# qpc001/ORB_SLAM2_Commit

Hardware: AMD Instinct MI355X
Metric: frames/sec ORB extract+match (2k kp) + LocalBA iters/sec, KITTI-00 stereo (higher is better)
Workload: dtype u8; 1 GPU; KITTI-00 stereo 1241x376, 2000 features, extract L+R + ComputeStereoMatches; batch_frames_per_gpu=256, global_batch_frames=256, nlevels=8, parallelism=frame-sharded x1, batches_in_flight=4

## Files before the change

### include/orbx_debug.h

```cpp
#ifndef ORBX_DEBUG_H
#define ORBX_DEBUG_H
#include "orbx.h"
#ifdef __cplusplus
extern "C" {
#endif

enum {
  ORBX_DBG_BLUR_LEVEL = 1,
  ORBX_DBG_CELL_COUNTS = 2,
  ORBX_DBG_CELL_TABLE = 3,
  ORBX_DBG_CANDIDATES = 4,
  ORBX_DBG_OCT_COUNTS = 5,
  ORBX_DBG_OCT_OUT = 6,
  ORBX_DBG_LEVEL_INFO = 7
};

long long orbx_debug_copy(orbx_extractor* h, int what, int image, int arg, void* dst, size_t cap);

enum {
  ORBX_LP_LEVELS = 1,
  ORBX_LP_RESIZE = 2,
  ORBX_LP_BOUNDS = 3,
  ORBX_LP_GRIDS = 4,
  ORBX_LP_REMAP = 5,
  ORBX_LP_XTAB = 6,
  ORBX_LP_YTAB = 7,
  ORBX_LP_PATH = 8
};
long long orbx_debug_launch_plan(const orbx_extractor_params* params, int width, int height, int what, int a0,
                                 int a1, int a2, long long* dst, size_t cap);

orbx_status orbx_debug_stereo_keypoints(orbx_extractor* left, orbx_extractor* right, const orbx_keypoint* kpsL,
                                        const uint8_t* descL, int nL, const orbx_keypoint* kpsR, const uint8_t* descR,
                                        int nR, float bf, float baseline, float* uRight, float* depth, int32_t* sad,
                                        int32_t* nmatches);
int orbx_debug_stereo_keypoints_check(const orbx_keypoint* kps, int n, int nlevels, int width, int height);

double orbx_debug_atan2_det(double y, double x);

int orbx_debug_lm_step(double state[5], int counts[2], double tempChi, double scale, int ok2, int cube_kind,
                       int ops);

int orbx_debug_exp(const double* x, int n, double* y, int device);
int orbx_debug_sim3_exp(const double update[7], const double S[8], int fix_scale, double out[8], int device);

int orbx_debug_log(const double* x, int n, double* y, int device);
int orbx_debug_acos(const double* x, int n, double* y, int device);
int orbx_debug_sim3_log(const double* S, int n, double* out, int32_t* branch, int device);
int orbx_debug_essgraph_linearize(const orbx_essential_graph_problem* problem, double* meas, double* err,
                                  double* J0, double* J1, double* H, double* b, int device);
int orbx_debug_essgraph_solve(const orbx_essential_graph_problem* problem, const double* H, const double* b,
                              double lambda, double* x, int32_t* ok, int device);
int orbx_debug_essgraph_phases(const orbx_essential_graph_problem* problem, const orbx_essential_graph_result* result,
                               double phase_ms[3], long long* envelope_blocks, int device);

int orbx_debug_ldlt(const double* S, const double* b, int N, double* x, int reps, float* ms);
int orbx_debug_ldlt_ex(const double* S, const double* b, int N, double* x, int reps, float* ms, int kind,
                       unsigned long long* stamps);

#define ORBX_BA_LDLT_AUTO 0
// ... 46 lines not shown
```

### orb_slam2_commit_amd/csrc/capi.hip

```cpp
#include <hip/hip_runtime.h>

#include <algorithm>
#include <cmath>
#include <cstring>
#include <map>
#include <memory>
#include <new>
#include <utility>
#include <string>
#include <vector>

#include "../../include/orbx.h"
#include "orbx_internal.h"
#include "orbx_scratch.h"
#include "orbx_stereo.h"
#include "orbx_prof.h"
#include "orbx_bow.h"

namespace orbx {
hipError_t upload_constants(const int* umax16, const int* gauss7);
hipError_t launch_blur(const Geometry& Gh, const Geometry* Gd, const int* tile_level, const BatchPtrs& B, int n_img,
                       hipStream_t st);
hipError_t launch_extract_stages(const Geometry& Gh, const Geometry* Gd, const CellInfo* cells, const int* tile_level,
                                 const LaunchPlan& LP, const BatchPtrs& B, int n_img, orbx_keypoint* kps, uint8_t* desc, int32_t* counts,
                                 int kp_cap, hipStream_t st, StageTimer* T);
size_t octree_smem_host(int NC, int cell_cap, int kcap);
hipError_t octree_set_smem_limit(size_t bytes);
}

using namespace orbx;

namespace {

inline int round_even(float v) { return (int)std::nearbyintf(v); }

constexpr size_t kInSlack = 4;

template <class T>
struct DevBuf {
  T* p = nullptr;
  size_t n = 0;
  ~DevBuf() { release(); }
  void release() {
    if (p) (void)hipFree(p);
    p = nullptr;
    n = 0;
  }
  hipError_t ensure(size_t count) {
    if (count <= n && p) return hipSuccess;
    release();
    size_t c = std::max<size_t>(count, 1);
    hipError_t e = hipMalloc((void**)&p, c * sizeof(T));
    if (e == hipSuccess) n = c;
    return e;
  }
};

struct Tables {
  std::vector<float> scale, inv_scale, sigma2, inv_sigma2;
  std::vector<int> nfeat;
// ... 220 lines not shown
        if (sx + 1 >= sw && sx >= sw - 1) { fx = 0; sx = sw - 1; }
        ResizeX X;
        X.sx0 = sx;
        X.sx1 = std::min(sx + 1, sw - 1);
        X.a0 = (int16_t)round_even((1.f - fx) * 2048);
        X.a1 = (int16_t)round_even(fx * 2048);
        if (sx + 1 >= sw) {
          X.a0 = 2048;
          X.a1 = 0;
        }
        P.xt.push_back(X);
      }
      L.ytab_off = (int)P.yt.size();
      for (int dy = 0; dy < dh; dy++) {
        float fy = (float)((dy + 0.5) * scale_y - 0.5);
        int sy = (int)std::floor(fy);
        fy -= sy;
        ResizeY Y;
        Y.sy0 = std::min(std::max(sy, 0), sh - 1);
        Y.sy1 = std::min(std::max(sy + 1, 0), sh - 1);
        Y.b0 = (int16_t)round_even((1.f - fy) * 2048);
        Y.b1 = (int16_t)round_even(fy * 2048);
        P.yt.push_back(Y);
      }
    }
  }
  {
    auto layout = [&](int wmax, int hmax, Geometry::FastGroup& g) {
      g.s = wmax + 6 <= 40 ? 40 : wmax + 6 <= 48 ? 48 : 80;
      g.rp = wmax <= 32 ? 2 : 1;
      g.tile_bytes = ((hmax + 6) * g.s + 15) & ~15;
      g.map_bytes = ((hmax + 2) * g.s + 15) & ~15;
      g.smem = g.tile_bytes + g.map_bytes + 2 * wmax * hmax;
    };
    constexpr int kFastLdsFit = 5 * 1024;
    int split = 0, wa = 1, ha = 1;
    for (int l = 0; l < p.nlevels; l++) {
      Geometry::FastGroup g{};
      layout(std::max(wa, lv_wmax[l]), std::max(ha, lv_hmax[l]), g);
      if (g.smem > kFastLdsFit) break;
      wa = std::max(wa, lv_wmax[l]);
      ha = std::max(ha, lv_hmax[l]);
      split = l + 1;
    }
    if (split == 0 || split == p.nlevels) split = p.nlevels;
    int wb = 1, hb = 1;
    for (int l = split; l < p.nlevels; l++) {
      wb = std::max(wb, lv_wmax[l]);
      hb = std::max(hb, lv_hmax[l]);
    }
    G.n_fg = 0;
    if (split == p.nlevels) {
      int w = 1, h = 1;
      for (int l = 0; l < p.nlevels; l++) {
        w = std::max(w, lv_wmax[l]);
        h = std::max(h, lv_hmax[l]);
      }
      layout(w, h, G.fg[0]);
      G.fg[0].c0 = 0;
      G.fg[0].c1 = (int)P.cells.size();
      G.n_fg = 1;
    } else {
      layout(wa, ha, G.fg[0]);
      G.fg[0].c0 = 0;
      G.fg[0].c1 = G.lv[split].cell_begin;
      layout(wb, hb, G.fg[1]);
      G.fg[1].c0 = G.lv[split].cell_begin;
      G.fg[1].c1 = (int)P.cells.size();
      G.n_fg = 2;
    }
  }
  G.rz_rows = 1;
  G.rz_stride = 16;
  for (int l = 1; l < G.nlevels; l++) {
    const LevelGeom& L = G.lv[l];
    P.rzb_x[l] = (int)P.rzb.size();
    for (int ox = 0; ox < L.w; ox += kRzTW) {
      const int sx0 = P.xt[L.xtab_off + ox].sx0, sx1 = P.xt[L.xtab_off + std::min(ox + kRzTW, L.w) - 1].sx1;
      P.rzb.push_back(make_int2(sx0, sx1));
      G.rz_stride = std::max(G.rz_stride, (sx1 - sx0 + 1 + 15) / 16 * 16);
    }
    P.rzb_y[l] = (int)P.rzb.size();
    for (int oy = 0; oy < L.h; oy += kRzTH) {
      const int sy0 = P.yt[L.ytab_off + oy].sy0, sy1 = P.yt[L.ytab_off + std::min(oy + kRzTH, L.h) - 1].sy1;
      P.rzb.push_back(make_int2(sy0, sy1));
      G.rz_rows = std::max(G.rz_rows, sy1 - sy0 + 1);
    }
  }
  if (G.rz_rows > kRzMaxRows || (size_t)G.rz_rows * (G.rz_stride + 2 * kRzTW) > 64 * 1024) return ORBX_ERR_SIZE;
  P.rzb_n = (int)P.rzb.size();
  for (int l = 1; l < G.nlevels; l++) {
    const LevelGeom& L = G.lv[l];
    P.strip[l] = strip_resize_ok(P, l);
    if (!P.strip[l]) continue;
    P.rsb_x[l] = (int)P.rzb.size();
    for (int ox = 0; ox < L.w; ox += kRsTW)
      P.rzb.push_back(make_int2(P.xt[L.xtab_off + ox].sx0, P.xt[L.xtab_off + std::min(ox + kRsTW, L.w) - 1].sx1));
    P.rsb_y[l] = (int)P.rzb.size();
    for (int oy = 0; oy < L.h; oy += kRsTH)
      P.rzb.push_back(make_int2(P.yt[L.ytab_off + oy].sy0, P.yt[L.ytab_off + std::min(oy + kRsTH, L.h) - 1].sy1));
  }
  G.rz_lc = 0;
  while ((1 << G.rz_lc) < G.rz_stride / 16) G.rz_lc++;
// ... 787 lines not shown
      break;
    }
    case ORBX_DBG_CANDIDATES: {
      std::vector<uint32_t> raw((size_t)G.cand_total);
      if (hipMemcpy(raw.data(), h->cand.p + (size_t)image * G.cand_total, raw.size() * 4, hipMemcpyDeviceToHost) !=
          hipSuccess)
        return ORBX_ERR_HIP;
      std::vector<uint32_t> logical;
      logical.reserve(raw.size());
      for (const CellInfo& c : P.cells)
        for (int q = 0; q < c.cap; q++) logical.push_back(raw[cell_slot(c, q)]);
      static_assert(sizeof(uint32_t) == sizeof(int), "host staging is int words");
      host.resize(logical.size());
      std::memcpy(host.data(), logical.data(), logical.size() * 4);
      device_src = false;
      break;
    }
    case ORBX_DBG_OCT_COUNTS:
      src = h->oct_count.p + (size_t)image * G.nlevels;
      bytes = sizeof(int) * G.nlevels;
      break;
    case ORBX_DBG_OCT_OUT:
      src = h->oct.p + (size_t)image * G.oct_total;
      bytes = sizeof(uint32_t) * G.oct_total;
      break;
    case ORBX_DBG_LEVEL_INFO:
      for (int l = 0; l < G.nlevels; l++) {
        const LevelGeom& L = G.lv[l];
        int v[8] = {L.w, L.h, L.cell_begin, L.cell_end, L.oct_off, L.oct_cap, L.nfeat, L.nIni};
        host.insert(host.end(), v, v + 8);
      }
      device_src = false;
      break;
    default:
      return ORBX_ERR_ARG;
  }
  if (!device_src) {
    bytes = host.size() * sizeof(int);
    if (dst) std::memcpy(dst, host.data(), std::min(bytes, cap));
    return (long long)bytes;
  }
  if (dst && cap) {
    if (hipMemcpy(dst, src, std::min(bytes, cap), hipMemcpyDeviceToHost) != hipSuccess) return ORBX_ERR_HIP;
  }
  return (long long)bytes;
}

extern "C" int orbx_debug_stereo_keypoints_check(const orbx_keypoint* kps, int n, int nlevels, int width,
                                                 int height) {
  if (n < 0 || (n > 0 && !kps) || nlevels < 1 || nlevels > kMaxLevelsPlan || width <= 0 || height <= 0)
    return ORBX_ERR_ARG;
  for (int i = 0; i < n; i++) {
    const orbx_keypoint& k = kps[i];
    if (k.octave < 0 || k.octave >= nlevels) return ORBX_ERR_ARG;
    if (!std::isfinite(k.x) || !std::isfinite(k.y) || std::signbit(k.x) || std::signbit(k.y)) return ORBX_ERR_ARG;
    if (!(k.x < (float)width) || !(k.y < (float)height)) return ORBX_ERR_ARG;
  }
  return ORBX_OK;
}

extern "C" orbx_status orbx_debug_stereo_keypoints(orbx_extractor* left, orbx_extractor* right,
                                                   const orbx_keypoint* kpsL, const uint8_t* descL, int nL,
                                                   const orbx_keypoint* kpsR, const uint8_t* descR, int nR, float bf,
                                                   float baseline, float* uRight, float* depth, int32_t* sad,
                                                   int32_t* nmatches) {
  if (!uRight || !depth || !sad || !nmatches || nL < 0 || nR < 0) return ORBX_ERR_ARG;
// ... 63 lines not shown
  }
  if (!params_ok(params) || width <= 0 || height <= 0) return ORBX_ERR_ARG;
  Plan P;
  const orbx_status s = build_plan(*params, make_tables(*params), width, height, P);
  if (s != ORBX_OK) return s;
  build_launch_plan(P, P.xt.data(), P.yt.data(), P.rzb.data(), P.LP);
  const Geometry& G = P.G;
  switch (what) {
    case ORBX_LP_LEVELS:
      for (int l = 0; l < G.nlevels; l++) {
        const LevelGeom& L = G.lv[l];
        out.insert(out.end(), {L.w, L.h, L.off, L.boff, L.bstride, L.tile_begin, L.tiles_x, L.tiles_y});
      }
      break;
    case ORBX_LP_RESIZE:
      for (int l = 1; l < G.nlevels; l++) {
        const ResizeDesc& D = P.LP.rz[l];
        out.insert(out.end(), {D.sw, D.sh, D.dw, D.dh, D.src_off, D.dst_off, D.pyr_bytes, D.X - P.xt.data(),
                               D.Y - P.yt.data(), D.bx - P.rzb.data(), D.by - P.rzb.data(), D.stride, D.rows, D.lc,
                               (D.dw + kRzTW - 1) / kRzTW, (D.dh + kRzTH - 1) / kRzTH});
      }
      break;
    case ORBX_LP_BOUNDS:
      for (int i = 0; i < P.rzb_n; i++) out.insert(out.end(), {P.rzb[i].x, P.rzb[i].y});
      break;
    case ORBX_LP_PATH:
      for (int l = 1; l < G.nlevels; l++) {
        const bool f = P.strip[l];
        const int tw = f ? kRsTW : kRzTW, th = f ? kRsTH : kRzTH;
        out.insert(out.end(), {f ? 1 : 0, (G.lv[l].w + tw - 1) / tw, (G.lv[l].h + th - 1) / th, tw, th,
                               f ? kRsStride : G.rz_stride, f ? kRsRows : G.rz_rows, f ? kRsR : 0});
      }
      break;
    case ORBX_LP_GRIDS: {
      if (a0 < 1) return ORBX_ERR_ARG;
      for (int l = 1; l < G.nlevels; l++)
        out.insert(out.end(), {(G.lv[l].w + kRzTW - 1) / kRzTW, (G.lv[l].h + kRzTH - 1) / kRzTH, a0});
      out.insert(out.end(), {G.ntiles, a0, 1});
      break;
    }
    case ORBX_LP_XTAB:
    case ORBX_LP_YTAB: {
      if (a0 < 1 || a0 >= G.nlevels) return ORBX_ERR_ARG;
      const LevelGeom& L = G.lv[a0];
      if (what == ORBX_LP_XTAB)
        for (int i = 0; i < L.w; i++) {
          const ResizeX& X = P.xt[L.xtab_off + i];
          out.insert(out.end(), {X.sx0, X.sx1, X.a0, X.a1});
        }
      else
        for (int i = 0; i < L.h; i++) {
          const ResizeY& Y = P.yt[L.ytab_off + i];
          out.insert(out.end(), {Y.sy0, Y.sy1, Y.b0, Y.b1});
        }
      break;
    }
    default:
      return ORBX_ERR_ARG;
  }
  return done();
}

typedef unsigned int u32x4 __attribute__((ext_vector_type(4)));
__global__ __launch_bounds__(256) void k_hbm_copy(u32x4* __restrict__ dst, const u32x4* __restrict__ src, size_t n) {
  const size_t i = (size_t)blockIdx.x * 256 + threadIdx.x;
  if (i < n) __builtin_nontemporal_store(__builtin_nontemporal_load(src + i), dst + i);
// ... 27 lines not shown
```

### orb_slam2_commit_amd/csrc/extract.hip

```cpp
#include <hip/hip_runtime.h>

#include <utility>

#include "orbx_device.h"
#include "orbx_internal.h"
#include "orbx_prof.h"

namespace orbx {

__constant__ float c_pattern_f[1024] = {
#include "brief_pattern_31.inc"
};
__constant__ uint4 c_icmask[64];
__constant__ double c_sincos[23] = {
    6.36619772367581382433e-01,
    1.57079632673412561417e+00,
    6.07710050650619224932e-11,
    1.0 / 51090942171709440000.0, -1.0 / 121645100408832000.0, 1.0 / 355687428096000.0,
    -1.0 / 1307674368000.0,       1.0 / 6227020800.0,           -1.0 / 39916800.0,
    1.0 / 362880.0,               -1.0 / 5040.0,                1.0 / 120.0,
    -1.0 / 6.0,
    1.0 / 2432902008176640000.0,  -1.0 / 6402373705728000.0,    1.0 / 20922789888000.0,
    -1.0 / 87178291200.0,         1.0 / 479001600.0,            -1.0 / 3628800.0,
    1.0 / 40320.0,                -1.0 / 720.0,                 1.0 / 24.0,
// ... 352 lines not shown
  RZ_PROBE_WRITE(ts1 - ts0, 0, ts2 - ts1, ts3 - ts2, 1);
}

__constant__ int c_gauss[7];

__device__ __forceinline__ int reflect101(int p, int n) {
  if (n == 1) return 0;
  while ((unsigned)p >= (unsigned)n) p = p < 0 ? -p : 2 * n - 2 - p;
  return p;
}

constexpr int kBIn = kBlurTileW + 16;
constexpr int kBStrip = 16;
#ifndef ORBX_BLUR_WPE
#define ORBX_BLUR_WPE 7
#endif
__global__ __launch_bounds__(BS, ORBX_BLUR_WPE) void k_blur(const Geometry* __restrict__ G, const int* __restrict__ tile_level,
                                                            BatchPtrs B, XcdRemap R) {
  constexpr int TR = kBlurTileH + 6;
  __shared__ __align__(16) uint8_t tin[(TR + 1) * kBIn];
  const int2 bi = xcd_block2(R);
  const int tile = bi.x, img = bi.y, tid = threadIdx.x;
  const int l = tile_level[tile];
  const LevelGeom& L = G->lv[l];
  const int t = tile - L.tile_begin;
  const int x0 = (t % L.tiles_x) * kBlurTileW, y0 = (t / L.tiles_x) * kBlurTileH;
  const uint8_t* src = level_ptr(*G, B, img, l);
  uint8_t* dst = B.blur + (size_t)img * G->blur_bytes + L.boff;
  const int w = L.w, h = L.h, bs = L.bstride;
  {
    constexpr int CPR = kBIn / 16, NQ = TR * CPR, KQ = (NQ + BS - 1) / BS;
    const __amdgpu_buffer_rsrc_t rs = __builtin_amdgcn_make_buffer_rsrc((void*)src, (short)0, w * h, 0x00020000);
    uint32_t v[KQ][4];
#pragma unroll
    for (int k = 0; k < KQ; k++) {
      const int q = k * BS + tid;
      const int ty = q / CPR, j = q - ty * CPR;
      v[k][0] = v[k][1] = v[k][2] = v[k][3] = 0;
      if (q < NQ) {
        const int sy = reflect101(y0 - 3 + ty, h);
        const int o = sy * w + x0 - 4 + 16 * j;
        if (o >= 0 && o + 16 <= w * h) {
          const auto r = __builtin_amdgcn_raw_buffer_load_b128(rs, o, 0, 0);
          v[k][0] = r[0];
          v[k][1] = r[1];
          v[k][2] = r[2];
          v[k][3] = r[3];
        } else {
#pragma unroll
          for (int b = 0; b < 16; b++)
            v[k][b >> 2] |= (uint32_t)__builtin_amdgcn_raw_buffer_load_b8(rs, o + b, 0, 0) << (8 * (b & 3));
        }
      }
    }
#pragma unroll
    for (int k = 0; k < KQ; k++) {
      const int q = k * BS + tid;
      const int ty = q / CPR, j = q - ty * CPR;
      if (q < NQ) *(uint4*)&tin[ty * kBIn + 16 * j] = make_uint4(v[k][0], v[k][1], v[k][2], v[k][3]);
    }
  }
  const bool left = x0 < 3, right = x0 + kBlurTileW + 3 > w;
  if (left || right) {
    __syncthreads();
    const int nfix = TR * 6;
    uint8_t vals[(TR * 6 + BS - 1) / BS];
#pragma unroll
    for (int k = 0; k < (TR * 6 + BS - 1) / BS; k++) {
      const int q = k * BS + tid;
      vals[k] = 0;
      if (q < nfix) {
        const int ty = q / 6, s = q - ty * 6;
        const int x = s < 3 ? -3 + s : w + (s - 3);
        const int c = x - (x0 - 4);
        if (c >= 0 && c < kBIn && (s < 3 ? left : right)) vals[k] = tin[ty * kBIn + reflect101(x, w) - (x0 - 4)];
      }
    }
    __syncthreads();
#pragma unroll
    for (int k = 0; k < (TR * 6 + BS - 1) / BS; k++) {
      const int q = k * BS + tid;
      if (q < nfix) {
        const int ty = q / 6, s = q - ty * 6;
        const int x = s < 3 ? -3 + s : w + (s - 3);
        const int c = x - (x0 - 4);
        if (c >= 0 && c < kBIn && (s < 3 ? left : right)) tin[ty * kBIn + c] = vals[k];
      }
    }
  }
  __syncthreads();
  const int g = tid & (kBlurTileW / 4 - 1);
  const int ys = (tid / (kBlurTileW / 4)) * kBStrip;
// ... 132 lines not shown
  constexpr int o[8] = {6 * S + 3, 5 * S + 5, 3 * S + 6, S + 5, 3, S + 1, 3 * S, 5 * S + 1};
  const int v = t[3 * S + 3];
  int p[8], lo2[8], hi2[8];
#pragma unroll
  for (int k = 0; k < 8; k++) p[k] = t[o[k]];
#pragma unroll
  for (int k = 0; k < 8; k++) lo2[k] = min(p[k], p[(k + 1) & 7]), hi2[k] = max(p[k], p[(k + 1) & 7]);
  int bl = 0, bh = 255;
#pragma unroll
  for (int k = 0; k < 8; k++) bl = max(bl, min(lo2[k], lo2[(k + 2) & 7])), bh = min(bh, max(hi2[k], hi2[(k + 2) & 7]));
  return bl > v + th || bh < v - th;
}
#endif

typedef short s16x2 __attribute__((ext_vector_type(2)));
__device__ __forceinline__ s16x2 as_s16x2(int v) { return __builtin_bit_cast(s16x2, v); }
__device__ __forceinline__ int as_int(s16x2 v) { return __builtin_bit_cast(int, v); }

__device__ __forceinline__ int lane_rank(uint64_t m) {
  return (int)__builtin_amdgcn_mbcnt_hi((uint32_t)(m >> 32), __builtin_amdgcn_mbcnt_lo((uint32_t)m, 0u));
}

#ifdef ORBX_FAST_PROBE
__device__ unsigned int* fast_probe_buf;
#define FAST_TS(k) const unsigned long long ts##k = __builtin_amdgcn_s_memtime()
#else
#define FAST_TS(k)
#endif

#ifndef ORBX_FAST_CPW
#define ORBX_FAST_CPW 2
#endif
constexpr int kFastCPW = ORBX_FAST_CPW;
template <int S, int RP>
__global__ __launch_bounds__(64) void k_fast(const Geometry* __restrict__ G, const CellInfo* __restrict__ cells,
                                             BatchPtrs B, int grp, XcdRemap R) {
  extern __shared__ __align__(16) uint8_t fast_smem[];
  const int tile_bytes = G->fg[grp].tile_bytes, map_bytes = G->fg[grp].map_bytes;
  uint8_t* tile = fast_smem;
  uint8_t* smap = fast_smem + tile_bytes;
  uint16_t* list = (uint16_t*)(fast_smem + tile_bytes + map_bytes);
  const int2 bi = xcd_block2(R);
  const int img = bi.y, lane = threadIdx.x;
  constexpr int CPR = (S + 15) / 16, RPI = 64 / CPR;
  constexpr int KMAX = (kMaxCell + 6 + RPI - 1) / RPI;
  const int lr = lane / CPR, lj = lane - lr * CPR;
  const bool lane_ok = lr < RPI;
  auto load_window = [&](const CellInfo& cc, uint32_t (&w)[KMAX][4]) {
    const uint8_t* lvl =
        cc.level == 0 ? B.in + (size_t)img * B.in_pitch : B.pyr + (size_t)img * G->pyr_bytes + cc.loff;
    const uint8_t* base = lvl + (size_t)(cc.y0 - 3) * cc.lw + (cc.x0 - 3);
    const int th = cc.y1 - cc.y0 + 7;
    const __amdgpu_buffer_rsrc_t rs =
        __builtin_amdgcn_make_buffer_rsrc((void*)base, (short)0, th * cc.lw + S, 0x00020000);
#pragma unroll
    for (int k = 0; k < KMAX; k++) {
      const int r = k * RPI + lr;
      const uint32_t off = (lane_ok && r < th) ? (uint32_t)(r * cc.lw + 16 * lj) : 0x80000000u;
      const auto q = __builtin_amdgcn_raw_buffer_load_b128(rs, off, 0, 0);
      w[k][0] = q[0];
      w[k][1] = q[1];
      w[k][2] = q[2];
      w[k][3] = q[3];
    }
  };
  const int cell0 = G->fg[grp].c0 + bi.x * kFastCPW, cend = G->fg[grp].c1;
  CellInfo cn = cells[cell0];
  uint32_t vn[KMAX][4];
  load_window(cn, vn);
#pragma unroll
  for (int q = 0; q < kFastCPW; q++) {
  const int cell = cell0 + q;
  if (cell >= cend) break;
  const CellInfo c = cn;
  uint32_t v[KMAX][4];
#pragma unroll
  for (int k = 0; k < KMAX; k++)
#pragma unroll
// ... 1 lines not shown
  if (q + 1 < kFastCPW && cell + 1 < cend) {
    cn = cells[cell + 1];
    load_window(cn, vn);
  }
  const int W = c.x1 - c.x0 + 1, H = c.y1 - c.y0 + 1, TH = H + 6;
  FAST_TS(0);
  if (q > 0) __syncthreads();
  {
    for (int i = lane * 16; i < map_bytes; i += 64 * 16) *(uint4*)(smap + i) = make_uint4(0, 0, 0, 0);
#pragma unroll
    for (int k = 0; k < KMAX; k++) {
      const int r = k * RPI + lr;
      if (k * RPI < TH && lane_ok && r < TH) {
        if constexpr (S % 16 == 0) {
          *(uint4*)(tile + r * S + 16 * lj) = make_uint4(v[k][0], v[k][1], v[k][2], v[k][3]);
        } else {
          if (16 * lj + 8 <= S) *(uint2*)(tile + r * S + 16 * lj) = make_uint2(v[k][0], v[k][1]);
          if (16 * lj + 16 <= S) *(uint2*)(tile + r * S + 16 * lj + 8) = make_uint2(v[k][2], v[k][3]);
        }
      }
    }
  }
  __syncthreads();
  const int ini = min(max(G->ini_th, 0), 255), mint = min(max(G->min_th, 0), 255);
  const int ly = RP == 2 ? (lane >> 5) : 0, lx = RP == 2 ? (lane & 31) : lane;
  const int cw = lx - W;
  constexpr int QU = 8 / RP;
#ifdef ORBX_FAST_PROBE
  unsigned long long ts_mid = 0;
  int n_compass = 0, n_even8 = 0, n_corner_ini = 0;
#endif
  auto detect = [&](int th) -> int {
    int n = 0;
    for (int y0r = 0; y0r < H; y0r += QU * RP) {
      const int eb = (y0r + ly) * S + lx;
      int cv[QU], c0[QU], c4[QU], c8[QU], c12[QU];
#pragma unroll
      for (int u = 0; u < QU; u++) {
        const uint8_t* t = tile + eb + u * RP * S;
        cv[u] = t[3 * S + 3];
        c0[u] = t[6 * S + 3];
        c4[u] = t[3 * S + 6];
        c8[u] = t[3];
        c12[u] = t[3 * S];
      }
#pragma unroll
      for (int u = 0; u < QU; u++) {
        const int hi = min(max(c0[u], c8[u]), max(c4[u], c12[u]));
        const int lo = max(min(c0[u], c8[u]), min(c4[u], c12[u]));
        const int v = max(hi - cv[u], cv[u] - lo) - (th + 1);
        const bool hit = (~v & cw & (y0r + u * RP + ly - H)) < 0;
        const uint64_t m = __ballot(hit);
        if (hit) list[n + lane_rank(m)] = (uint16_t)(eb + u * RP * S);
        n += __popcll(m);
      }
    }
    __syncthreads();
#ifdef ORBX_FAST_PROBE
    if (th == ini) ts_mid = __builtin_amdgcn_s_memtime(), n_compass = n;
#endif
    int nc = 0;
    for (int i0 = 0; i0 < n; i0 += 64) {
      const int i = i0 + lane;
      int e = 0, sc1 = 0;
      bool corner = false;
      if (i < n) {
        e = list[i];
        sc1 = ring_score1<S>(tile + e);
        corner = sc1 > th;
      }
#ifdef ORBX_FAST_PROBE
      if (th == ini) n_even8 += __popcll(__ballot(i < n && even8_test<S>(tile + e, th)));
#endif
      const uint64_t m = __ballot(corner);
      __syncthreads();
      if (corner) {
        list[nc + lane_rank(m)] = (uint16_t)e;
        smap[e + S + 1] = (uint8_t)sc1;
      }
      nc += __popcll(m);
    }
    __syncthreads();
    return nc;
  };
  auto keep = [&](int e, int thr) -> bool {
    const uint8_t* m = smap + e;
    const int s = m[S + 1];
    const int n0 = m[0], n1 = m[1], n2 = m[2], n3 = m[S], n4 = m[S + 2], n5 = m[2 * S], n6 = m[2 * S + 1],
              n7 = m[2 * S + 2];
// ... 28 lines not shown
  int pos = 0;
  for (int i0 = 0; i0 < nc; i0 += 64) {
    const int i = i0 + lane;
    int e = 0;
    bool k = false;
    if (i < nc) {
      const int le = list[i];
      e = le & 0x7FFF;
      k = cnt > 0 ? (le >> 15) != 0 : keep(e, thr);
    }
    const uint64_t m = __ballot(k);
    if (k) {
      const int p = pos + lane_rank(m);
      const int y = e / S, x = e - y * S;
      if (p < c.cap)
      {
        const uint32_t v = ((uint32_t)(smap[e + S + 1] - 1) << 24) | ((uint32_t)(c.y0 + y) << 12) | (uint32_t)(c.x0 + x);
        if (p < kin) out_in[p]= v; else out[p] = v;
      }
    }
    pos += __popcll(m);
  }
  if (lane == 0) B.cell_count[(size_t)img * G->ncells + cell] = min(pos, c.cap);
#ifdef ORBX_FAST_PROBE
  FAST_TS(5);
  if (lane < 8 && fast_probe_buf) {
    const unsigned long long t[8] = {ts1 - ts0, ts_mid - ts1, ts2 - ts_mid, ts3 - ts2, ts4 - ts3, ts5 - ts4,
                                     (unsigned long long)((cnt == 0) | (n_corner_ini << 1) | (cnt << 16)),
                                     (unsigned long long)(n_compass | (n_even8 << 16))};
    fast_probe_buf[((size_t)img * G->ncells + cell) * 8 + lane] = (unsigned int)t[lane];
  }
#endif
  }
}

struct OctSmem {
  int16_t* x0;
  int16_t* y0;
  int16_t* x1;
  int16_t* y1;
  int* cnt;
  int* seq;
  int* ccnt;
  int16_t* cidx;
  int16_t* nidx;
  int* sa;
  int* sb;
  uint64_t* key;
  int* cpre;
  int* ctrl;
  uint32_t* kp;
  uint16_t* kn;
};

__host__ __device__ inline int next_pow2(int v) {
  int p = 1;
  while (p < v) p <<= 1;
  return p;
}

__host__ __device__ inline size_t octree_smem_bytes(int NC, int cell_cap, int kcap) {
  const int NP2 = next_pow2(NC);
  size_t b = 0;
  b += 2 * 4 * NC * sizeof(int16_t);
  b += 2 * 2 * NC * sizeof(int);
  b += NC * 4 * sizeof(int);
// ... 396 lines not shown
    oct_out[i] = ((uint32_t)(key >> 56) << 24) | (uint32_t)(key & 0xFFFFFF);
  }
  if (tid == 0) *oct_cnt = nout;
#ifdef ORBX_OCT_PROBE
  if (tid == 0 && oct_probe_buf) {
    const unsigned long long ot3 = __builtin_amdgcn_s_memtime();
    unsigned int* o = oct_probe_buf + ((size_t)img * G->nlevels + l) * 8;
    o[0] = (unsigned int)(ot1 - ot0);
    o[1] = (unsigned int)(ot2 - ot1);
    o[2] = (unsigned int)ot_p1;
    o[3] = (unsigned int)n_p1;
    o[4] = (unsigned int)ot_p2;
    o[5] = (unsigned int)n_p2;
    o[6] = (unsigned int)(ot3 - ot0);
    o[7] = (unsigned int)T;
  }
#endif
}

__device__ __forceinline__ int wave_sum_dpp(int v) {
  v += __builtin_amdgcn_update_dpp(0, v, 0x111, 0xF, 0xF, true);
  v += __builtin_amdgcn_update_dpp(0, v, 0x112, 0xF, 0xF, true);
  v += __builtin_amdgcn_update_dpp(0, v, 0x114, 0xF, 0xF, true);
  v += __builtin_amdgcn_update_dpp(0, v, 0x118, 0xF, 0xF, true);
  return __builtin_amdgcn_readlane(v, 15) + __builtin_amdgcn_readlane(v, 31) + __builtin_amdgcn_readlane(v, 47) +
         __builtin_amdgcn_readlane(v, 63);
}


constexpr int kPatchR = 18;
constexpr int kPatchRows = 2 * kPatchR + 1;
constexpr int kPS = 80;
constexpr int kDescLds = kPatchRows * kPS + 256;
__constant__ uint8_t c_patch_slot[128] = {0,1,4,5,8,9,10,12,13,14,16,17,18,20,21,22,24,25,26,28,29,30,32,33,34,36,37,38,40,41,42,43,44,45,46,47,48,49,50,51,52,53,54,55,56,57,58,59,60,61,62,63,64,65,66,67,68,69,70,71,72,73,74,75,76,77,78,79,80,81,82,83,84,85,86,87,88,89,90,91,92,93,94,95,96,97,98,99,100,101,102,103,104,105,106,107,108,109,110,112,113,114,116,117,118,120,121,122,124,125,126,128,129,130,132,133,134,136,137,138,140,141,144,145,255,255,255,255};
__constant__ int c_patch_hw[kPatchRows] = {6,  8,  10, 11, 12, 13, 14, 15, 16, 16, 17, 17, 18, 18, 18, 18, 18, 18, 18,
                                           18, 18, 18, 18, 18, 18, 17, 17, 16, 16, 15, 14, 13, 12, 11, 10, 8,  6};

#ifndef ORBX_DESC_K
#define ORBX_DESC_K 8
#endif
constexpr int kDescK = ORBX_DESC_K;
static_assert(kDescK * 8 <= 64, "one descriptor dword per lane");

template <class F, int... I>
__device__ __forceinline__ void static_for_impl(F&& f, std::integer_sequence<int, I...>) {
  (f(std::integral_constant<int, I>{}), ...);
}
template <int N, class F>
__device__ __forceinline__ void static_for(F&& f) {
  static_for_impl(f, std::make_integer_sequence<int, N>{});
}
__device__ __forceinline__ const uint8_t* lane_ptr(const uint8_t* p, int j) {
  const uint64_t a = (uint64_t)p;
  const uint32_t lo = __builtin_amdgcn_readlane((uint32_t)a, j), hi = __builtin_amdgcn_readlane((uint32_t)(a >> 32), j);
  return (const uint8_t*)(((uint64_t)hi << 32) | lo);
}
__device__ __forceinline__ float lane_f(float v, int j) {
  return __builtin_bit_cast(float, __builtin_amdgcn_readlane(__builtin_bit_cast(int, v), j));
}

__global__ __launch_bounds__(BS) void k_describe(const Geometry* __restrict__ G, BatchPtrs B,
                                                 orbx_keypoint* __restrict__ kps, uint8_t* __restrict__ desc,
                                                 int32_t* __restrict__ counts, int kp_cap, XcdRemap R) {
  __shared__ __align__(16) uint8_t s_desc[BS / 64][kDescLds];
  const int2 bi = xcd_block2(R);
  const int img = bi.y;
  const int lane = threadIdx.x & 63, wv = threadIdx.x >> 6;
  const int i0 = __builtin_amdgcn_readfirstlane((bi.x * (BS / 64) + wv) * kDescK);
  const int nl = G->nlevels;
// ... 21 lines not shown
    acc += cnt[ll];
  }
  const LevelGeom& L = G->lv[l];
  const uint32_t v = B.oct[(size_t)img * G->oct_total + L.oct_off + (i - first)];
  const int w = L.w, h = L.h;
  const float lscale = L.scale, lsize = L.kp_size;
  const int x = v & 0xFFF, y = (v >> 12) & 0xFFF, score = v >> 24;
  const uint8_t* lvl = level_ptr(*G, B, img, l);
  const uint8_t* icp = lvl + (size_t)(y - 15) * w + (x - 15);

  const int r = lane >> 1, hh = lane & 1;
  uint32_t q[kDescK][4];
#pragma unroll
  for (int j = 0; j < kDescK; j++) {
    const int wj = __builtin_amdgcn_readlane(w, j);
    const __amdgpu_buffer_rsrc_t rs =
        __builtin_amdgcn_make_buffer_rsrc((void*)lane_ptr(icp, j), (short)0, 31 * wj, 0x00020000);
    const uint32_t off = lane < 62 ? (uint32_t)(r * wj + 16 * hh) : 0x80000000u;
    const auto t = __builtin_amdgcn_raw_buffer_load_b128(rs, off, 0, 0);
    q[j][0] = t[0];
    q[j][1] = t[1];
    q[j][2] = t[2];
    q[j][3] = t[3];
  }
  constexpr int kPatchLd = 2;
  const int bs = L.bstride;
  const int x0 = (x - kPatchR) & ~15;
  const uint8_t* pbl = B.blur + (size_t)img * G->blur_bytes + L.boff;
  constexpr int PS = kPS;
  const uint32_t corr_l = (uint32_t)(kPatchR * PS + (x - x0)) - (0x400000u * (uint32_t)PS + 0x4B400000u);
  int srow[kPatchLd], skk[kPatchLd], shw[kPatchLd];
#pragma unroll
  for (int k = 0; k < kPatchLd; k++) {
    const int e = c_patch_slot[lane + 64 * k];
    srow[k] = e == 0xFF ? -1 : e >> 2;
    skk[k] = e & 3;
    shw[k] = c_patch_hw[e == 0xFF ? 0 : e >> 2];
  }
  uint32_t pv[2][kPatchLd][4];
  int pdst[2][kPatchLd];
  auto load_patch = [&](int j, uint32_t (&dst)[kPatchLd][4], int (&dofs)[kPatchLd]) {
    const int bt8 = __builtin_amdgcn_readlane(bs, j) * 8, hj = __builtin_amdgcn_readlane(h, j);
    const int xj = __builtin_amdgcn_readlane(x, j), y0j = __builtin_amdgcn_readlane(y, j) - kPatchR;
    const int aj = (xj - kPatchR) & 15, tx0 = (xj - kPatchR) >> 4;
    const __amdgpu_buffer_rsrc_t rs =
        __builtin_amdgcn_make_buffer_rsrc((void*)lane_ptr(pbl, j), (short)0, ((hj + 7) >> 3) * bt8, 0x00020000);
#pragma unroll
    for (int k = 0; k < kPatchLd; k++) {
      const int lo = (kPatchR + aj - shw[k]) >> 4, hi = (kPatchR + aj + shw[k]) >> 4;
      const int ch = lo + skk[k];
      const bool ok = srow[k] >= 0 && ch <= hi;
      const int yy = y0j + srow[k];
      const uint32_t off = ok ? (uint32_t)((yy >> 3) * bt8 + (tx0 + ch) * 128 + (yy & 7) * 16) : 0x80000000u;
      dofs[k] = ok ? srow[k] * kPS + 16 * ch : -1;
      const auto t = __builtin_amdgcn_raw_buffer_load_b128(rs, off, 0, 0);
      dst[k][0] = t[0];
      dst[k][1] = t[1];
      dst[k][2] = t[2];
      dst[k][3] = t[3];
    }
  };
  load_patch(0, pv[0], pdst[0]);
  if (kDescK > 1) load_patch(1, pv[1], pdst[1]);
  int M01 = 0, M10 = 0;
  {
    const uint4 mk = c_icmask[lane];
    static_for<kDescK>([&](auto jc) {
      constexpr int j = decltype(jc)::value;
      const uint32_t I0 = q[j][0] & mk.x, I1 = q[j][1] & mk.y, I2 = q[j][2] & mk.z, I3 = q[j][3] & mk.w;
      uint32_t s0 = __builtin_amdgcn_udot4(I0, 0x01010101u, 0u, false);
// ... 104 lines not shown
  for (int l = 1; l < Gh.nlevels; l++) {
    const int tw = LP.rz[l].strip ? kRsTW : kRzTW, th = LP.rz[l].strip ? kRsTH : kRzTH;
    rz_grid[l] = dim3((Gh.lv[l].w + tw - 1) / tw, (Gh.lv[l].h + th - 1) / th, n_img);
    rz[l] = LP.rz[l];
#ifdef ORBX_RZ_PROBE
    rz[l].level = l;
    rz[l].probe_base = l == 1 ? 0 : rz[l - 1].probe_base + (int)(rz_grid[l - 1].x * rz_grid[l - 1].y * rz_grid[l - 1].z);
#endif
    if (!make_xcd_remap(rz_grid[l].x, rz_grid[l].y, rz_grid[l].z, &rz[l].rm)) return hipErrorInvalidValue;
  }
  for (int g = 0; g < Gh.n_fg; g++) {
    const Geometry::FastGroup& F = Gh.fg[g];
    if (F.c1 <= F.c0) continue;
    fast_grid[g] = dim3((F.c1 - F.c0 + kFastCPW - 1) / kFastCPW, n_img);
    if (!make_xcd_remap(fast_grid[g].x, fast_grid[g].y, 1, &fast_rm[g])) return hipErrorInvalidValue;
  }
  XcdRemap blur_rm;
  if (!make_xcd_remap(Gh.ntiles, n_img, 1, &blur_rm) || !make_xcd_remap(max(nb, 1), n_img, 1, &desc_rm))
    return hipErrorInvalidValue;
  for (int l = 1; l < Gh.nlevels; l++) {
    T->begin(st);
    if (rz[l].strip)
      hipLaunchKernelGGL(k_resize_strip, rz_grid[l], dim3(BS), 0, st, rz[l], B.in, B.in_pitch, B.pyr);
    else
      hipLaunchKernelGGL(k_resize, rz_grid[l], dim3(BS), (size_t)Gh.rz_rows * (Gh.rz_stride + 2 * kRzTW), st, rz[l], B.in,
                         B.in_pitch, B.pyr);
    T->end(ST_RESIZE, st);
  }
  if (Gh.ncells > 0) {
    T->begin(st);
    for (int g = 0; g < Gh.n_fg; g++) {
      const Geometry::FastGroup& F = Gh.fg[g];
      if (F.c1 <= F.c0) continue;
      auto kf = F.s == 40   ? (F.rp == 2 ? k_fast<40, 2> : k_fast<40, 1>)
                : F.s == 48 ? (F.rp == 2 ? k_fast<48, 2> : k_fast<48, 1>)
                            : k_fast<80, 1>;
      hipLaunchKernelGGL(kf, fast_grid[g], dim3(64), F.smem, st, Gd, cells, B, g, fast_rm[g]);
    }
    T->end(ST_FAST, st);
  } else {
    (void)hipMemsetAsync(B.oct_count, 0, sizeof(int) * Gh.nlevels * n_img, st);
  }
  {
    T->begin(st);
    hipLaunchKernelGGL(k_blur, dim3(Gh.ntiles, n_img), dim3(BS), 0, st, Gd, tile_level, B, blur_rm);
    T->end(ST_BLUR, st);
  }
  if (Gh.ncells > 0) {
    T->begin(st);
    const bool one = n_img <= kOctOneLaunch;
    for (int gi = 0; gi < (one ? 1 : Gh.n_og); gi++) {
      const OctGroup& og = one ? Gh.og_all : Gh.og[gi];
      const size_t smem = octree_smem_bytes(og.node_cap, og.cell_cap, og.kcap);
      if (og.nt == 512)
        hipLaunchKernelGGL(k_octree<512>, dim3(n_img, og.l1 - og.l0), dim3(512), smem, st, Gd, cells, B, og);
      else
        hipLaunchKernelGGL(k_octree<256>, dim3(n_img, og.l1 - og.l0), dim3(256), smem, st, Gd, cells, B, og);
    }
    T->end(ST_OCTREE, st);
  }
  T->begin(st);
  hipLaunchKernelGGL(k_describe, dim3(max(nb, 1), n_img), dim3(BS), 0, st, Gd, B, kps, desc, counts, kp_cap, desc_rm);
  T->end(ST_DESCRIBE, st);
  return hipGetLastError();
}

size_t octree_smem_host(int NC, int cell_cap, int kcap) { return octree_smem_bytes(NC, cell_cap, kcap); }

hipError_t octree_set_smem_limit(size_t bytes) {
// ... 27 lines not shown
```

### orb_slam2_commit_amd/csrc/orbx_internal.h

```cpp
#pragma once
#include <hip/hip_runtime.h>
#include <stdint.h>

#include "../../include/orbx.h"
#include "orbx_device.h"

namespace orbx {

constexpr int kMaxLevelsPlan = 16;
constexpr int kEdgeThresholdHost = 19;

struct LevelGeom {
  int w, h;
  long long off;
  long long boff;
  int bstride;
  int minBX, minBY, maxBX, maxBY;
  int cell_begin, cell_end;
  int cand_begin, cand_cap;
  int nfeat;
  int nIni;
  float hX;
  int oct_off, oct_cap;
  float scale;
  float kp_size;
  int xtab_off, ytab_off;
  int tile_begin, tiles_x, tiles_y;
};

constexpr int kOctOneLaunch = 2;
struct OctGroup {
  int l0, l1, nt;
  int node_cap;
  int cell_cap;
  int kcap;
};

struct Geometry {
  int nlevels, width, height;
  int ini_th, min_th;
  LevelGeom lv[kMaxLevelsPlan];
  long long pyr_bytes, blur_bytes;
  int ncells, cand_total, oct_total, max_kps, ntiles;
  int node_cap;
  int cell_cap;
  int oct_kcap;
  OctGroup og[2];
  int n_og;
  OctGroup og_all;
  struct FastGroup {
    int c0, c1, s, rp, tile_bytes, map_bytes, smem;
  } fg[2];
  int n_fg;
  int rz_rows;
  int rz_stride;
  int rz_lc;
};

constexpr int kRzTW = 128, kRzTH = 32;
constexpr int kRzMaxRows = 64;

#ifndef ORBX_RS_R
#define ORBX_RS_R 8
#endif
constexpr int kRsR = ORBX_RS_R;
constexpr int kRsTW = 256, kRsTH = 4 * kRsR;
constexpr int kRsStride = 336;
constexpr int kRsRows = kRsTH * 5 / 4 + 3;

struct CellInfo {
  int16_t level, kin;
  int16_t x0, y0, x1, y1;
  int cand_off, cap;
  int lw, loff;
  int ovf_off;
};
__host__ __device__ inline int cell_slot(const CellInfo& c, int p) {
  return p < c.kin ? c.cand_off + p : c.ovf_off + (p - c.kin);
}

struct ResizeX {
  int sx0, sx1;
  int16_t a0, a1;
};
// ... 54 lines not shown
```

Before: 113,700 frames/s.

## Size FAST window registers per group and trim blur/FAST tail work

The FAST kernel gains a template parameter for the number of window load chunks, computed on the host from each group's actual tile height instead of the worst-case cell height. This cuts register arrays and unrolled loads. The detect loop now splits into full unrolled trips plus one partial tail trip, so rows past the tile are not processed. The blur tile loader skips global loads and LDS stores for rows and columns beyond the image edge. The patch slot table is generated at compile time. More kernel instantiations are added, and a new size check can reject geometries that need more chunks than the available variants.

```diff
diff --git a/include/orbx_debug.h b/include/orbx_debug.h
--- a/include/orbx_debug.h
+++ b/include/orbx_debug.h
@@ -12,7 +12,8 @@
   ORBX_DBG_CANDIDATES = 4,
   ORBX_DBG_OCT_COUNTS = 5,
   ORBX_DBG_OCT_OUT = 6,
-  ORBX_DBG_LEVEL_INFO = 7
+  ORBX_DBG_LEVEL_INFO = 7,
+  ORBX_DBG_PATCH_SLOTS = 8
 };
 
 long long orbx_debug_copy(orbx_extractor* h, int what, int image, int arg, void* dst, size_t cap);
@@ -25,7 +26,8 @@
   ORBX_LP_REMAP = 5,
   ORBX_LP_XTAB = 6,
   ORBX_LP_YTAB = 7,
-  ORBX_LP_PATH = 8
+  ORBX_LP_PATH = 8,
+  ORBX_LP_FAST = 9
 };
 long long orbx_debug_launch_plan(const orbx_extractor_params* params, int width, int height, int what, int a0,
                                  int a1, int a2, long long* dst, size_t cap);
diff --git a/orb_slam2_commit_amd/csrc/capi.hip b/orb_slam2_commit_amd/csrc/capi.hip
--- a/orb_slam2_commit_amd/csrc/capi.hip
+++ b/orb_slam2_commit_amd/csrc/capi.hip
@@ -26,6 +26,7 @@
                                  int kp_cap, hipStream_t st, StageTimer* T);
 size_t octree_smem_host(int NC, int cell_cap, int kcap);
 hipError_t octree_set_smem_limit(size_t bytes);
+const uint8_t* patch_slot_table();
 }
 
 using namespace orbx;
@@ -312,6 +313,8 @@
       g.tile_bytes = ((hmax + 6) * g.s + 15) & ~15;
       g.map_bytes = ((hmax + 2) * g.s + 15) & ~15;
       g.smem = g.tile_bytes + g.map_bytes + 2 * wmax * hmax;
+      const int rpi = 64 / ((g.s + 15) / 16);
+      g.nk = std::max(g.s == 80 ? 4 : 2, (hmax + 6 + rpi - 1) / rpi);
     };
     constexpr int kFastLdsFit = 5 * 1024;
     int split = 0, wa = 1, ha = 1;
@@ -349,6 +352,8 @@
       G.fg[1].c1 = (int)P.cells.size();
       G.n_fg = 2;
     }
+    for (int g = 0; g < G.n_fg; g++)
+      if (G.fg[g].nk > (G.fg[g].s == 80 ? 5 : 3)) return ORBX_ERR_SIZE;
   }
   G.rz_rows = 1;
   G.rz_stride = 16;
@@ -1202,6 +1207,10 @@
       }
       device_src = false;
       break;
+    case ORBX_DBG_PATCH_SLOTS:
+      host.assign(patch_slot_table(), patch_slot_table() + 128);
+      device_src = false;
+      break;
     default:
       return ORBX_ERR_ARG;
   }
@@ -1331,6 +1340,12 @@
                                f ? kRsStride : G.rz_stride, f ? kRsRows : G.rz_rows, f ? kRsR : 0});
       }
       break;
+    case ORBX_LP_FAST:
+      for (int g = 0; g < G.n_fg; g++) {
+        const Geometry::FastGroup& F = G.fg[g];
+        out.insert(out.end(), {F.c0, F.c1, F.s, F.rp, F.nk, F.tile_bytes, F.map_bytes, F.smem});
+      }
+      break;
     case ORBX_LP_GRIDS: {
       if (a0 < 1) return ORBX_ERR_ARG;
       for (int l = 1; l < G.nlevels; l++)
diff --git a/orb_slam2_commit_amd/csrc/extract.hip b/orb_slam2_commit_amd/csrc/extract.hip
--- a/orb_slam2_commit_amd/csrc/extract.hip
+++ b/orb_slam2_commit_amd/csrc/extract.hip
@@ -408,12 +408,13 @@
     constexpr int CPR = kBIn / 16, NQ = TR * CPR, KQ = (NQ + BS - 1) / BS;
     const __amdgpu_buffer_rsrc_t rs = __builtin_amdgcn_make_buffer_rsrc((void*)src, (short)0, w * h, 0x00020000);
     uint32_t v[KQ][4];
+    const int ty_last = min(kBlurTileH, h - y0) + 5, j_last = (w + 2 - (x0 - 4)) >> 4;
 #pragma unroll
     for (int k = 0; k < KQ; k++) {
       const int q = k * BS + tid;
       const int ty = q / CPR, j = q - ty * CPR;
       v[k][0] = v[k][1] = v[k][2] = v[k][3] = 0;
-      if (q < NQ) {
+      if (q < NQ && ty <= ty_last && j <= j_last) {
         const int sy = reflect101(y0 - 3 + ty, h);
         const int o = sy * w + x0 - 4 + 16 * j;
         if (o >= 0 && o + 16 <= w * h) {
@@ -433,7 +434,8 @@
     for (int k = 0; k < KQ; k++) {
       const int q = k * BS + tid;
       const int ty = q / CPR, j = q - ty * CPR;
-      if (q < NQ) *(uint4*)&tin[ty * kBIn + 16 * j] = make_uint4(v[k][0], v[k][1], v[k][2], v[k][3]);
+      if (q < NQ && ty <= ty_last && j <= j_last)
+        *(uint4*)&tin[ty * kBIn + 16 * j] = make_uint4(v[k][0], v[k][1], v[k][2], v[k][3]);
     }
   }
   const bool left = x0 < 3, right = x0 + kBlurTileW + 3 > w;
@@ -632,7 +634,7 @@
 #define ORBX_FAST_CPW 2
 #endif
 constexpr int kFastCPW = ORBX_FAST_CPW;
-template <int S, int RP>
+template <int S, int RP, int NK>
 __global__ __launch_bounds__(64) void k_fast(const Geometry* __restrict__ G, const CellInfo* __restrict__ cells,
                                              BatchPtrs B, int grp, XcdRemap R) {
   extern __shared__ __align__(16) uint8_t fast_smem[];
@@ -643,7 +645,8 @@
   const int2 bi = xcd_block2(R);
   const int img = bi.y, lane = threadIdx.x;
   constexpr int CPR = (S + 15) / 16, RPI = 64 / CPR;
-  constexpr int KMAX = (kMaxCell + 6 + RPI - 1) / RPI;
+  constexpr int KMAX = NK;
+  static_assert(NK >= 1 && NK <= (kMaxCell + 6 + RPI - 1) / RPI, "no window is taller than kMaxCell + 6 rows");
   const int lr = lane / CPR, lj = lane - lr * CPR;
   const bool lane_ok = lr < RPI;
   auto load_window = [&](const CellInfo& cc, uint32_t (&w)[KMAX][4]) {
@@ -711,11 +714,13 @@
 #endif
   auto detect = [&](int th) -> int {
     int n = 0;
-    for (int y0r = 0; y0r < H; y0r += QU * RP) {
+    auto trip = [&](int y0r, auto fullc, int nu) {
+      constexpr bool full = decltype(fullc)::value;
       const int eb = (y0r + ly) * S + lx;
       int cv[QU], c0[QU], c4[QU], c8[QU], c12[QU];
 #pragma unroll
       for (int u = 0; u < QU; u++) {
+        if (!full && u >= nu) break;
         const uint8_t* t = tile + eb + u * RP * S;
         cv[u] = t[3 * S + 3];
         c0[u] = t[6 * S + 3];
@@ -725,6 +730,7 @@
       }
 #pragma unroll
       for (int u = 0; u < QU; u++) {
+        if (!full && u >= nu) break;
         const int hi = min(max(c0[u], c8[u]), max(c4[u], c12[u]));
         const int lo = max(min(c0[u], c8[u]), min(c4[u], c12[u]));
         const int v = max(hi - cv[u], cv[u] - lo) - (th + 1);
@@ -733,7 +739,10 @@
         if (hit) list[n + lane_rank(m)] = (uint16_t)(eb + u * RP * S);
         n += __popcll(m);
       }
-    }
+    };
+    int y0r = 0;
+    for (; y0r + QU * RP <= H; y0r += QU * RP) trip(y0r, std::true_type{}, QU);
+    if (y0r < H) trip(y0r, std::false_type{}, (H - y0r + RP - 1) / RP);
     __syncthreads();
 #ifdef ORBX_FAST_PROBE
     if (th == ini) ts_mid = __builtin_amdgcn_s_memtime(), n_compass = n;
@@ -828,6 +837,11 @@
   }
 #endif
   }
+}
+
+template <int S, int RP, int N0>
+static auto fast_kernel(int nk) -> decltype(&k_fast<S, RP, N0>) {
+  return nk <= N0 ? k_fast<S, RP, N0> : k_fast<S, RP, N0 + 1>;
 }
 
 struct OctSmem {
@@ -1290,9 +1304,43 @@
 constexpr int kPatchRows = 2 * kPatchR + 1;
 constexpr int kPS = 80;
 constexpr int kDescLds = kPatchRows * kPS + 256;
-__constant__ uint8_t c_patch_slot[128] = {0,1,4,5,8,9,10,12,13,14,16,17,18,20,21,22,24,25,26,28,29,30,32,33,34,36,37,38,40,41,42,43,44,45,46,47,48,49,50,51,52,53,54,55,56,57,58,59,60,61,62,63,64,65,66,67,68,69,70,71,72,73,74,75,76,77,78,79,80,81,82,83,84,85,86,87,88,89,90,91,92,93,94,95,96,97,98,99,100,101,102,103,104,105,106,107,108,109,110,112,113,114,116,117,118,120,121,122,124,125,126,128,129,130,132,133,134,136,137,138,140,141,144,145,255,255,255,255};
-__constant__ int c_patch_hw[kPatchRows] = {6,  8,  10, 11, 12, 13, 14, 15, 16, 16, 17, 17, 18, 18, 18, 18, 18, 18, 18,
-                                           18, 18, 18, 18, 18, 18, 17, 17, 16, 16, 15, 14, 13, 12, 11, 10, 8,  6};
+struct PatchHW {
+  int v[kPatchRows];
+};
+constexpr PatchHW kPatchHW = {{6,  8,  10, 11, 12, 13, 14, 15, 16, 16, 17, 17, 18, 18, 18, 18, 18, 18, 18,
+                               18, 18, 18, 18, 18, 18, 17, 17, 16, 16, 15, 14, 13, 12, 11, 10, 8,  6}};
+__constant__ PatchHW c_patch_hw = kPatchHW;
+struct PatchSlots {
+  uint8_t e[128];
+};
+constexpr int patch_row_chunks(int r) {
+  int m = 0;
+  for (int a = 0; a < 16; a++) {
+    const int n = ((kPatchR + a + kPatchHW.v[r]) >> 4) - ((kPatchR + a - kPatchHW.v[r]) >> 4) + 1;
+    m = n > m ? n : m;
+  }
+  return m;
+}
+constexpr PatchSlots make_patch_slots() {
+  PatchSlots t{};
+  for (int s = 0; s < 128; s++) t.e[s] = 0xFF;
+  int n = 0, nrest = 0;
+  uint8_t rest[12] = {};
+  for (int ch = 0; ch < 4; ch++) {
+    int rows[kPatchRows] = {}, nr = 0;
+    for (int r = 0; r < kPatchRows; r++)
+      if (patch_row_chunks(r) > ch) rows[nr++] = r;
+    for (int q = 0; q + 4 <= nr; q += 4)
+      for (int i = 0; i < 4; i++) t.e[n++] = (uint8_t)(rows[q + i] << 2 | ch);
+    for (int q = nr & ~3; q < nr; q++) rest[nrest++] = (uint8_t)(rows[q] << 2 | ch);
+  }
+  for (int i = 0; i < nrest; i++) t.e[n++] = rest[i];
+  return t;
+}
+constexpr PatchSlots kPatchSlots = make_patch_slots();
+static_assert(kPatchSlots.e[123] != 0xFF && kPatchSlots.e[124] == 0xFF, "124 patch slots: two loads per lane");
+__constant__ PatchSlots c_patch_slot = kPatchSlots;
+const uint8_t* patch_slot_table() { return kPatchSlots.e; }
 
 #ifndef ORBX_DESC_K
 #define ORBX_DESC_K 8
@@ -1380,10 +1428,10 @@
   int srow[kPatchLd], skk[kPatchLd], shw[kPatchLd];
 #pragma unroll
   for (int k = 0; k < kPatchLd; k++) {
-    const int e = c_patch_slot[lane + 64 * k];
+    const int e = c_patch_slot.e[lane + 64 * k];
     srow[k] = e == 0xFF ? -1 : e >> 2;
     skk[k] = e & 3;
-    shw[k] = c_patch_hw[e == 0xFF ? 0 : e >> 2];
+    shw[k] = c_patch_hw.v[e == 0xFF ? 0 : e >> 2];
   }
   uint32_t pv[2][kPatchLd][4];
   int pdst[2][kPatchLd];
@@ -1554,9 +1602,9 @@
     for (int g = 0; g < Gh.n_fg; g++) {
       const Geometry::FastGroup& F = Gh.fg[g];
       if (F.c1 <= F.c0) continue;
-      auto kf = F.s == 40   ? (F.rp == 2 ? k_fast<40, 2> : k_fast<40, 1>)
-                : F.s == 48 ? (F.rp == 2 ? k_fast<48, 2> : k_fast<48, 1>)
-                            : k_fast<80, 1>;
+      auto kf = F.s == 40   ? (F.rp == 2 ? fast_kernel<40, 2, 2>(F.nk) : fast_kernel<40, 1, 2>(F.nk))
+                : F.s == 48 ? fast_kernel<48, 1, 2>(F.nk)
+                            : fast_kernel<80, 1, 4>(F.nk);
       hipLaunchKernelGGL(kf, fast_grid[g], dim3(64), F.smem, st, Gd, cells, B, g, fast_rm[g]);
     }
     T->end(ST_FAST, st);
diff --git a/orb_slam2_commit_amd/csrc/orbx_internal.h b/orb_slam2_commit_amd/csrc/orbx_internal.h
--- a/orb_slam2_commit_amd/csrc/orbx_internal.h
+++ b/orb_slam2_commit_amd/csrc/orbx_internal.h
@@ -50,6 +50,7 @@
   OctGroup og_all;
   struct FastGroup {
     int c0, c1, s, rp, tile_bytes, map_bytes, smem;
+    int nk;
   } fg[2];
   int n_fg;
   int rz_rows;
```

Result: faster. 115,200 frames/s, median of 6 (+1.4%).
